# AcherStyx/SSD-Object-Detection

Hardware: AMD Instinct MI355X
Metric: images/sec SSD300 train step, batch 64 (higher is better)
Workload: dtype bf16; 1 GPU; BASELINE configs[2]: SSD300 full train step (anchor match+encode, image normalisation, conv fwd, loss, conv bwd, per-variable clip (64 variables) + Adam), per-GPU batch 64, 80 classes, synthetic COCO-shaped boxes; per_gpu_batch=64, global_batch=64, parallelism=single

## Files before the change

### ssd-object-detection_amd/csrc/conv.hip

```cpp
#include <atomic>
#include <cstdint>
#include <type_traits>
#include "common.h"
#include <hip/hip_bf16.h>
#include <stdlib.h>

#include "conv_common.h"
namespace {

template <int EPI>
__global__ void k_igemm_finalize(ConvGeom g, Epilogue ep) {
    const int n4 = (g.N + 3) >> 2;
    const long long idx = (long long)blockIdx.x * blockDim.x + threadIdx.x;
    if (idx >= (long long)g.M * n4) return;
    const int m = (int)(idx / n4), n = (int)(idx - (long long)m * n4) * 4;
    const bool full = n + 3 < g.N;
    float v[4] = {0.f, 0.f, 0.f, 0.f};
    if (full && !(g.N & 3)) {
        for (int z = 0; z < ep.ksplit; ++z) {
            const float4 t = *reinterpret_cast<const float4*>(ep.slab + ((long long)z * g.M + m) * g.N + n);
            v[0] += t.x; v[1] += t.y; v[2] += t.z; v[3] += t.w;
        }
    } else {
        for (int z = 0; z < ep.ksplit; ++z) {
// ... 362 lines not shown
    else keep_frags(fx, FW_);                                                                                       \
    __builtin_amdgcn_sched_barrier(0);                                                                              \
    __builtin_amdgcn_s_setprio(0);                                                                                  \
    if constexpr (!(ABL & 2)) __builtin_amdgcn_s_barrier();                                                              \
    __builtin_amdgcn_sched_barrier(0);

    for (int t = 0; t < nt; ++t) {
        const int cb = (t & 1) * BUF, nb = BUF - cb;
#pragma unroll
        for (int c = 0; c < 2; ++c) { fw0[c][0] = ldf(cb + OFF_W0 + wf0 + c * 2048); fw0[c][1] = ldf(cb + OFF_W0 + wf1 + c * 2048); }
        __builtin_amdgcn_sched_barrier(0);
#pragma unroll
        for (int p = 0; p < 4; ++p) { fx[p][0] = ldf(cb + OFF_X0 + xf0 + p * 2048); fx[p][1] = ldf(cb + OFF_X0 + xf1 + p * 2048); }
        __builtin_amdgcn_sched_barrier(0);
        asm volatile("s_waitcnt lgkmcnt(8)" ::: "memory");
        if constexpr (!(ABL & 1)) issue_x(nb + OFF_X1, 1);
        advance_x();
        SSD_PHASE_MMA(0, 0, fw0)
#pragma unroll
        for (int c = 0; c < 2; ++c) { fw1[c][0] = ldf(cb + OFF_W1 + wf0 + c * 2048); fw1[c][1] = ldf(cb + OFF_W1 + wf1 + c * 2048); }
        if constexpr (!(ABL & 1)) issue_w(cb + OFF_W0, 0);
        SSD_PHASE_MMA(0, 1, fw1)
#pragma unroll
        for (int p = 0; p < 4; ++p) { fx[p][0] = ldf(cb + OFF_X1 + xf0 + p * 2048); fx[p][1] = ldf(cb + OFF_X1 + xf1 + p * 2048); }
        if constexpr (!(ABL & 1)) issue_x(cb + OFF_X0, 0);
        SSD_PHASE_MMA(1, 1, fw1)
        if constexpr (!(ABL & 1)) issue_w(cb + OFF_W1, 1);
        wq += 8;
        asm volatile("s_waitcnt vmcnt(6)" ::: "memory");
        SSD_PHASE_MMA(1, 0, fw0)
    }
#undef SSD_PHASE_MMA
    if (wr == 0) __builtin_amdgcn_s_barrier();

    if (staged_ok<EPI>(g, ep) && !(g.ablate & 8)) {
        asm volatile("s_waitcnt vmcnt(0)" ::: "memory");
        auto row_to_m = [&](int row) { const int m = m0 + row; return m < g.M ? m : -1; };
        staged_epilogue<EPI, 256, 256, 4, 8, 512>(acc, smem, g, ep, n0, wr * 128, wc * 64, tid, row_to_m);
        return;
    }
    int mrow[8];
#pragma unroll
    for (int p = 0; p < 8; ++p) {
        const int m = m0 + wr * 128 + p * 16 + (lane & 15);
        mrow[p] = m < g.M ? m : -1;
    }
    conv_epilogue_rows<EPI, 4, 8>(acc, g, ep, mrow, n0 + wc * 64, lane);
}

constexpr int P32_PITCH = 96;
constexpr int P32_PATCH = 32 * 1024;
constexpr int EPI_NO_PREFETCH = 256;
constexpr int P32_OFF_MAP = 2 * P32_PATCH;

template <int BN, int EPI, bool FLAT>
__global__ __launch_bounds__(512) __attribute__((amdgpu_waves_per_eu(4, 4))) void k_conv3x3_patch32(
    const bf16_raw* __restrict__ x, const bf16_raw* __restrict__ w, ConvGeom g, Epilogue ep, int tiles_x, int tiles_y, int nblocks, int rowflat) {
    constexpr int CT = BN / 32;
    constexpr int PT = 4;
    constexpr int WBYTES = BN * 64;
    constexpr int OFF_W = 2 * P32_PATCH;
    constexpr int OFF_DUMMY = OFF_W + 2 * WBYTES;
    extern __shared__ __attribute__((aligned(16))) char smem[];

    const int tid = threadIdx.x, lane = tid & 63;
    const int wave = __builtin_amdgcn_readfirstlane(tid >> 6);
    const int wave_m = wave & 3, wave_n = wave >> 2;
    const int ntn = (g.N + BN - 1) / BN;
    const int kx = blockIdx.x >> 3;
    const int pblock = (kx / ntn) * 8 + (blockIdx.x & 7);
    if (pblock >= nblocks) return;
    const int n0 = (kx % ntn) * BN;
    constexpr bool flat = FLAT;
    const int Q = FLAT ? g.W + 1 : PATCH_W;
    const int img = (g.H + 1) * Q;
    int b = 0, y0 = 0, x0 = 0, f0 = 0;
    if constexpr (FLAT) {
        f0 = pblock * 256;
    } else {
        int t = pblock;
        const int tx = t % tiles_x; t /= tiles_x;
        x0 = tx * 16;
        if (rowflat) { y0 = t * 16; }
        else { const int ty = t % tiles_y; b = t / tiles_y; y0 = ty * 16; }
    }
    auto image_row = [&](int r) {
        if (!rowflat) { const int y = y0 + r; return (unsigned)y < (unsigned)g.H ? b * g.H + y : -1; }
        const int R = y0 + r;
        if (R < 0) return -1;
        const int bb = fdiv(R, g.d_h1), yy = R - bb * g.d_h1.d;
        return (bb < g.B && yy < g.H) ? bb * g.H + yy : -1;
    };
    auto flat_pixel = [&](int f) {
        if (f < 0) return -1;
        const int bb = f / img;
        const int r = f - bb * img;
        const int yy = r / Q, xx = r - yy * Q - 1;
        return (bb < g.B && yy < g.H && (unsigned)xx < (unsigned)g.W) ? (bb * g.H + yy) * g.W + xx : -1;
    };

    const __amdgpu_buffer_rsrc_t xres = __builtin_amdgcn_make_buffer_rsrc((void*)x, 0, (unsigned)g.B * g.H * g.W * g.C * 2u, 0x00020000);
    const __amdgpu_buffer_rsrc_t wres = __builtin_amdgcn_make_buffer_rsrc((void*)w, 0, (unsigned)g.N * (unsigned)g.ldw * 2u, 0x00020000);
    constexpr unsigned OOB = 0xfffffff0u;
    unsigned pvo[4];
#pragma unroll
    for (int j = 0; j < 4; ++j) {
// ... 102 lines not shown
            }
        }
    } else {
    dma_patch(0, 0);
    dma_w(0, 0, 0);
    for (int chunk = 0; chunk < nchunk; ++chunk) {
        const int pb = (chunk & 1) * P32_PATCH;
        const bool next_chunk = chunk + 1 < nchunk;
#pragma unroll
        for (int tap = 0; tap < 9; ++tap) {
            const int wb = ((chunk + tap) & 1) * WBYTES;
            if (tap == 1 && next_chunk) asm volatile("s_waitcnt vmcnt(4) lgkmcnt(0)" ::: "memory");
            else asm volatile("s_waitcnt vmcnt(0) lgkmcnt(0)" ::: "memory");
            __builtin_amdgcn_s_barrier();
            if (!(g.ablate & 16)) {
                if (tap < 8) dma_w(chunk, tap + 1, ((chunk + tap + 1) & 1));
                else if (next_chunk) dma_w(chunk + 1, 0, ((chunk + tap + 1) & 1));
            }
            if (tap == 0 && next_chunk && !(g.ablate & 32)) dma_patch(chunk + 1, (chunk + 1) & 1);
            bf16x8_t fx[PT], fw[CT];
            const int tapoff = pb + xbase + ((tap / 3) * Q + tap % 3) * P32_PITCH;
#pragma unroll
            for (int p = 0; p < PT; ++p) fx[p] = ldf(tapoff + p * prow);
#pragma unroll
            for (int c = 0; c < CT; ++c) fw[c] = ldf(wb + wbase + c * 1024);
            __builtin_amdgcn_s_setprio(0);
#pragma unroll
            for (int c = 0; c < CT; ++c)
#pragma unroll
                for (int p = 0; p < PT; ++p)
                    acc[c][p] = __builtin_amdgcn_mfma_f32_16x16x32_bf16(fw[c], fx[p], acc[c][p], 0, 0, 0);
            __builtin_amdgcn_s_setprio(3);
        }
    }
    }
    if (staged_ok<EPI>(g, ep) && !(g.ablate & 8)) {
        auto row_to_m = [&](int row) {
            if (flat) return flat_pixel(f0 + row);
            const int ir = image_row(row >> 4), xx = x0 + (row & 15);
            return (ir >= 0 && xx < g.Wo) ? ir * g.Wo + xx : -1;
        };
        auto pool_index = [&](int py, int px) -> long long {
            if (flat) return -1;
            int bb = b, gy = (y0 >> 1) + py;
            const int gx = (x0 >> 1) + px;
            if (rowflat) {
                const int R = y0 + 2 * py;
                bb = fdiv(R, g.d_h1);
                gy = (R - bb * g.d_h1.d) >> 1;
                if (bb >= g.B) return -1;
            }
            return (gy < ep.pool_h && gx < ep.pool_w) ? ((long long)bb * ep.pool_h + gy) * ep.pool_w + gx : -1;
        };
        if constexpr (FLAT && (BN == 128 || EPI == EPI_DGRAD)) {
            LdsSide<P32_OFF_MAP, -1, -1> side;
            side.map = side.fill = !(g.ablate & EPI_NO_PREFETCH);
            side.signs = side.bias = false;
            staged_epilogue<EPI, 256, BN, CT, PT, 512>(acc, smem, g, ep, n0, wave_m * 64, wave_n * (16 * CT), tid, row_to_m, pool_index, side);
        } else {
            staged_epilogue<EPI, 256, BN, CT, PT, 512>(acc, smem, g, ep, n0, wave_m * 64, wave_n * (16 * CT), tid, row_to_m, pool_index);
        }
        return;
    }
    int mrow[PT];
#pragma unroll
    for (int p = 0; p < PT; ++p) {
        if (flat) {
            mrow[p] = flat_pixel(f0 + (4 * wave_m + p) * 16 + (lane & 15));
        } else {
            const int ir = image_row(4 * wave_m + p), xx = x0 + (lane & 15);
            mrow[p] = (ir >= 0 && xx < g.Wo) ? ir * g.Wo + xx : -1;
        }
    }
    conv_epilogue_rows<EPI, CT, PT>(acc, g, ep, mrow, n0 + wave_n * (16 * CT), lane);
}

constexpr int P5_PIX = 34 * PATCH_W;
constexpr int P5_NDMA = (P5_PIX * 6 + 63) / 64;
constexpr int P5_PATCH = P5_NDMA * 1024;
constexpr int P5_WSLOT = 128 * 64;
constexpr int P5_OFF_W = 2 * P5_PATCH;
constexpr int P5_OFF_DUMMY = P5_OFF_W + 4 * P5_WSLOT;
constexpr int P5_LOOP_LDS = P5_OFF_DUMMY + 1024;
constexpr int P5_OFF_SIGNS = P5_LOOP_LDS;
constexpr int P5_OFF_MAP = P5_OFF_SIGNS + 512 * 16;
constexpr int P5_OFF_BIAS = P5_OFF_MAP + 512 * 4;
constexpr int P5_LDS = P5_OFF_BIAS + 128 * 4;
static_assert(P5_LDS <= 160 * 1024, "k_conv3x3_p512: LDS of one workgroup");

template <int EPI, bool FLAT>
__global__ __launch_bounds__(512) void k_conv3x3_p512(const bf16_raw* __restrict__ x, const bf16_raw* __restrict__ w, ConvGeom g,
                                                      Epilogue ep, int tiles_x, int tiles_y, int nblocks, int rowflat) {
    constexpr int BN = 128, CT = 4, PT = 8;
    extern __shared__ __attribute__((aligned(16))) char smem[];
    const int tid = threadIdx.x, lane = tid & 63;
    const int wave = __builtin_amdgcn_readfirstlane(tid >> 6);
    const int wave_m = wave & 3, wave_n = wave >> 2;
    const int ntn = (g.N + BN - 1) / BN;
    const int kx = blockIdx.x >> 3;
    const int pblock = (kx / ntn) * 8 + (blockIdx.x & 7);
    if (pblock >= nblocks) return;
    const int n0 = (kx % ntn) * BN;
    const int Q = FLAT ? g.W + 1 : PATCH_W;
    const int img = (g.H + 1) * Q;
    int b = 0, y0 = 0, x0 = 0, f0 = 0;
    if constexpr (FLAT) {
        f0 = pblock * 512;
    } else {
        int t = pblock;
        const int tx = t % tiles_x; t /= tiles_x;
        x0 = tx * 16;
        if (rowflat) { y0 = t * 32; }
        else { const int ty = t % tiles_y; b = t / tiles_y; y0 = ty * 32; }
    }
    auto image_row = [&](int r) {
        if (!rowflat) { const int y = y0 + r; return (unsigned)y < (unsigned)g.H ? b * g.H + y : -1; }
        const int R = y0 + r;
        if (R < 0) return -1;
        const int bb = fdiv(R, g.d_h1), yy = R - bb * g.d_h1.d;
        return (bb < g.B && yy < g.H) ? bb * g.H + yy : -1;
    };
    auto flat_pixel = [&](int f) {
        if (f < 0) return -1;
        const int bb = f / img;
        const int r = f - bb * img;
        const int yy = r / Q, xx = r - yy * Q - 1;
        return (bb < g.B && yy < g.H && (unsigned)xx < (unsigned)g.W) ? (bb * g.H + yy) * g.W + xx : -1;
    };
    const __amdgpu_buffer_rsrc_t xres = __builtin_amdgcn_make_buffer_rsrc((void*)x, 0, (unsigned)g.B * g.H * g.W * g.C * 2u, 0x00020000);
    const __amdgpu_buffer_rsrc_t wres = __builtin_amdgcn_make_buffer_rsrc((void*)w, 0, (unsigned)g.N * (unsigned)g.ldw * 2u, 0x00020000);
    constexpr unsigned OOB = 0xfffffff0u;
    unsigned pvo[8];
#pragma unroll
    for (int j = 0; j < 8; ++j) {
        const int q = (wave + 8 * j) * 64 + lane;
        const int pp = q / 6, sl = q - pp * 6;
        int pix;
        if constexpr (FLAT) {
            pix = pp < 512 + 2 * (Q + 1) ? flat_pixel(f0 - (Q + 1) + pp) : -1;
        } else {
            const int py = pp / PATCH_W, px = pp - py * PATCH_W;
// ... 3 lines not shown
        }
        pvo[j] = (sl < 4 && pix >= 0 && wave + 8 * j < P5_NDMA) ? ((unsigned)pix * (unsigned)g.C + (unsigned)(sl * 8)) * 2u : OOB;
    }
    unsigned wvo;
    {
        const int row = 16 * wave + (lane >> 2);
        const int piece = (lane & 3) ^ ((-(row >> 2)) & 3);
        const int n = n0 + row;
        wvo = n < g.N ? ((unsigned)n * (unsigned)g.ldw + (unsigned)(piece * 8)) * 2u : OOB;
        if (g.ablate & 16) wvo = OOB;
    }
    const int nchunk = g.C >> 5;
    const int nstep = nchunk * 9;
    auto dma_piece = [&](int chunk, int buf, int j, bool live) {
        char* dst = wave + 8 * j < P5_NDMA ? smem + buf * P5_PATCH + (wave + 8 * j) * 1024 : smem + P5_OFF_DUMMY;
        __builtin_amdgcn_raw_ptr_buffer_load_lds(xres, (lds_void*)dst, 16, live ? pvo[j] : OOB, chunk * 64, 0, 0);
    };
    auto dma_w = [&](int step) {
        const int st = step < nstep ? step : nstep - 1;
        const int ch = st / 9, tp = st - ch * 9;
        __builtin_amdgcn_raw_ptr_buffer_load_lds(wres, (lds_void*)(smem + P5_OFF_W + (step & 3) * P5_WSLOT + wave * 1024), 16, wvo,
                                                 (tp * g.C + ch * 32) * 2, 0, 0);
    };
    f32x4_t acc[CT][PT];
#pragma unroll
    for (int c = 0; c < CT; ++c)
#pragma unroll
        for (int p = 0; p < PT; ++p) acc[c][p] = f32x4_t{0.f, 0.f, 0.f, 0.f};

    const int frow = lane & 15, fk = lane >> 4;
    const int xbase = (FLAT ? 8 * wave_m * 16 + frow : 8 * wave_m * PATCH_W + frow) * P32_PITCH + fk * 16;
    constexpr int prow = (FLAT ? 16 : PATCH_W) * P32_PITCH;
    int wbase;
    {
        const int row = wave_n * 64 + frow;
        wbase = P5_OFF_W + row * 64 + ((fk ^ ((-(row >> 2)) & 3)) << 4);
    }
    auto ldf = [&](int addr) { return lds_read_b128_scoped(smem + addr, smem); };
    auto load_x = [&](bf16x8_t (&fx)[PT], int pb, int tap) {
        const int tapoff = pb + xbase + ((tap / 3) * Q + tap % 3) * P32_PITCH;
#pragma unroll
        for (int p = 0; p < PT; ++p) fx[p] = ldf(tapoff + p * prow);
    };
    auto load_w = [&](bf16x8_t (&fw)[CT], int step) {
        const int wb = (step & 3) * P5_WSLOT;
#pragma unroll
        for (int c = 0; c < CT; ++c) fw[c] = ldf(wb + wbase + c * 1024);
    };
    auto row_to_m = [&](int row) {
        if constexpr (FLAT) return flat_pixel(f0 + row);
        const int ir = image_row(row >> 4), xx = x0 + (row & 15);
        return (ir >= 0 && xx < g.Wo) ? ir * g.Wo + xx : -1;
    };
    LdsSide<P5_OFF_MAP, P5_OFF_SIGNS, P5_OFF_BIAS> side;
    side.map = side.fill = !(g.ablate & EPI_NO_PREFETCH) && staged_ok<EPI>(g, ep);
    side.signs = side.bias = false;
    if constexpr (EPI == EPI_DGRAD) {
        const long long sign_bytes = (long long)g.M * (g.N >> 3);
        side.signs = side.map && ep.mask_bits && !ep.mask_src && (g.N & 127) == 0 &&
                     (reinterpret_cast<unsigned long long>(ep.mask_bits) & 15ull) == 0 && sign_bytes < (1ll << 31) - 16;
        if (side.signs) {
            const int m = row_to_m(tid);
            lds_st4_scoped(smem + P5_OFF_MAP + tid * 4, smem, m);
            side.fill = false;
            const __amdgpu_buffer_rsrc_t sres = __builtin_amdgcn_make_buffer_rsrc((void*)ep.mask_bits, 0, (unsigned)sign_bytes, 0x00020000);
            dma16_buf(sres, smem + P5_OFF_SIGNS + wave * 1024, m >= 0 ? (unsigned)m * (unsigned)(g.N >> 3) + (unsigned)(n0 >> 3) : OOB);
        }
    } else {
        side.bias = side.map;
        if (side.bias) {
            const __amdgpu_buffer_rsrc_t bres = __builtin_amdgcn_make_buffer_rsrc((void*)ep.bias, 0, ep.bias ? (unsigned)g.N * 4u : 0u, 0x00020000);
            const int n = n0 + wave * 64 + lane;
            char* dst = wave < 2 ? smem + P5_OFF_BIAS + wave * 256 : smem + P5_OFF_DUMMY;
            __builtin_amdgcn_raw_ptr_buffer_load_lds(bres, (lds_void*)dst, 4, (wave < 2 && n < g.N) ? (unsigned)n * 4u : OOB, 0, 0, 0);
        }
    }
#pragma unroll
    for (int j = 0; j < 8; ++j) dma_piece(0, 0, j, true);
    dma_w(0); dma_w(1); dma_w(2);
    bf16x8_t fxa[PT], fxb[PT], fwa[CT], fwb[CT];
    asm volatile("s_waitcnt vmcnt(2)" ::: "memory");
    __builtin_amdgcn_s_barrier();
    load_x(fxa, 0, 0);
    load_w(fwa, 0);
    auto run_chunk = [&](int chunk, auto par_tag) {
        constexpr int PAR = decltype(par_tag)::value;
        const int pb = (chunk & 1) * P5_PATCH;
        const bool next_chunk = chunk + 1 < nchunk && !(g.ablate & 32);
#pragma unroll
        for (int tap = 0; tap < 9; ++tap) {
            constexpr int NT[9] = {1, 3, 5, 5, 5, 3, 1, 1, 1};
            if (NT[tap] == 1) asm volatile("s_waitcnt vmcnt(1) lgkmcnt(0)" ::: "memory");
            else if (NT[tap] == 3) asm volatile("s_waitcnt vmcnt(3) lgkmcnt(0)" ::: "memory");
            else asm volatile("s_waitcnt vmcnt(5) lgkmcnt(0)" ::: "memory");
            __builtin_amdgcn_s_barrier();
            const int step = chunk * 9 + tap;
            dma_w(step + 3);
            if (tap < 4) {
                dma_piece(chunk + 1, (chunk + 1) & 1, 2 * tap, next_chunk);
                dma_piece(chunk + 1, (chunk + 1) & 1, 2 * tap + 1, next_chunk);
            }
            bf16x8_t (&fxc)[PT] = ((tap + PAR) & 1) ? fxb : fxa;
            bf16x8_t (&fxn)[PT] = ((tap + PAR) & 1) ? fxa : fxb;
            bf16x8_t (&fwc)[CT] = ((tap + PAR) & 1) ? fwb : fwa;
            bf16x8_t (&fwn)[CT] = ((tap + PAR) & 1) ? fwa : fwb;
            if (tap < 8) load_x(fxn, pb, tap + 1);
            else load_x(fxn, next_chunk ? (P5_PATCH - pb) : pb, next_chunk ? 0 : 8);
            load_w(fwn, step + 1 < nstep ? step + 1 : step);
#pragma unroll
            for (int c = 0; c < CT; ++c)
// ... 1019 lines not shown
```

### ssd-object-detection_amd/csrc/conv_common.h

```cpp
#pragma once
#include <atomic>
#include <cstdint>
#include <type_traits>
#include "common.h"
#include <hip/hip_bf16.h>

namespace {

typedef __attribute__((__vector_size__(8 * sizeof(__bf16)))) __bf16 bf16x8_t;
typedef __attribute__((__vector_size__(4 * sizeof(float)))) float f32x4_t;
typedef __attribute__((__vector_size__(4 * sizeof(short)))) short s16x4_t;
typedef unsigned short bf16_raw;

constexpr int WG = 256;

struct FastDiv {
    unsigned mg;
    int sh;
    int d;
};

inline FastDiv make_fastdiv(int d) {
    FastDiv f;
    f.d = d;
// ... 166 lines not shown
#pragma unroll
        for (int j = 0; j < 4; ++j) if (n + j < N) b4[j] = ep.bias[n + j];
    }
}

template <int EPI, int CT, int PT>
__device__ __forceinline__ void conv_epilogue_rows(f32x4_t (&acc)[CT][PT], const ConvGeom& g, const Epilogue& ep,
                                                   const int (&mrow)[PT], int nbase, int lane) {
#pragma unroll
    for (int c = 0; c < CT; ++c) {
        const int n = nbase + c * 16 + (lane >> 4) * 4;
        if (n >= g.N) continue;
        const bool full = n + 3 < g.N;
        if (ep.slab) {
            float* sl = ep.slab + (long long)blockIdx.y * g.M * g.N;
#pragma unroll
            for (int p = 0; p < PT; ++p) {
                const int m = mrow[p];
                if (m < 0) continue;
                float* o = sl + (long long)m * g.N + n;
                if (full && !(g.N & 3)) {
                    *reinterpret_cast<float4*>(o) = make_float4(acc[c][p][0], acc[c][p][1], acc[c][p][2], acc[c][p][3]);
                    continue;
                }
#pragma unroll
                for (int j = 0; j < 4; ++j) if (n + j < g.N) o[j] = acc[c][p][j];
            }
            continue;
        }
        float bias4[4];
        if constexpr (EPI == EPI_DGRAD) { bias4[0] = bias4[1] = bias4[2] = bias4[3] = 0.f; }
        else load_bias4(ep, n, g.N, full, bias4);
#pragma unroll
        for (int p = 0; p < PT; ++p) {
            const int m = mrow[p];
            if (m < 0) continue;
            float v[4] = {acc[c][p][0] + bias4[0], acc[c][p][1] + bias4[1], acc[c][p][2] + bias4[2], acc[c][p][3] + bias4[3]};
            epi_store<EPI>(v, m, n, full, g, ep);
        }
    }
}

template <int EPI>
__device__ __forceinline__ bool staged_ok(const ConvGeom& g, const Epilogue& ep) {
    if (ep.slab) return false;
    if constexpr (EPI == EPI_FWD) return (g.N & 7) == 0 && (ep.ldo & 7) == 0;
    if constexpr (EPI == EPI_DGRAD) return (g.N & 7) == 0 && (ep.ldo & 7) == 0;
    return true;
}

struct NoPool { __device__ long long operator()(int, int) const { return -1; } };

struct NoSide {
    static constexpr int MAP_OFF = -1, SIGN_OFF = -1, BIAS_OFF = -1;
    bool map = false, fill = false, signs = false, bias = false;
};
template <int MAP_OFF_, int SIGN_OFF_, int BIAS_OFF_>
struct LdsSide {
    static constexpr int MAP_OFF = MAP_OFF_, SIGN_OFF = SIGN_OFF_, BIAS_OFF = BIAS_OFF_;
    bool map;
    bool fill;
    bool signs;
    bool bias;
};

__device__ __forceinline__ uint4 lds_ld16_scoped(const char* __restrict__ p, const char* __restrict__ other) {
    (void)other;
    return *reinterpret_cast<const uint4*>(p);
}
__device__ __forceinline__ void lds_st16_scoped(char* __restrict__ p, const char* __restrict__ other, uint4 v) {
    (void)other;
    *reinterpret_cast<uint4*>(p) = v;
}
__device__ __forceinline__ void lds_st8_scoped(char* __restrict__ p, const char* __restrict__ other, uint2 v) {
    (void)other;
    *reinterpret_cast<uint2*>(p) = v;
}
__device__ __forceinline__ void lds_st4_scoped(char* __restrict__ p, const char* __restrict__ other, int v) {
    (void)other;
    *reinterpret_cast<int*>(p) = v;
}
__device__ __forceinline__ bf16x8_t lds_read_b128_scoped(const char* __restrict__ p, const char* __restrict__ other) {
    (void)other;
    return *reinterpret_cast<const bf16x8_t*>(p);
}
typedef __attribute__((address_space(3))) s16x4_t lds_s16x4;
__device__ __forceinline__ s16x4_t lds_read_tr16_scoped(const char* __restrict__ p, const char* __restrict__ other) {
    (void)other;
    return __builtin_amdgcn_ds_read_tr16_b64_v4i16((lds_s16x4*)p);
}

__device__ __attribute__((aligned(16))) const unsigned g_zero16[4] = {0u, 0u, 0u, 0u};

typedef __attribute__((address_space(3))) void lds_void;
typedef __attribute__((address_space(1))) const void gbl_void;

__device__ __forceinline__ void dma16_buf(__amdgpu_buffer_rsrc_t r, char* lds, unsigned off) {
    __builtin_amdgcn_raw_ptr_buffer_load_lds(r, (lds_void*)lds, 16, off, 0, 0, 0);
}

constexpr int PATCH_W = 18;
constexpr int PATCH_PIX = PATCH_W * PATCH_W;

template <int EPI, int BM, int BN, int NT, typename RowMap, typename PoolMap, bool DG_BATCHED = true, typename Side = NoSide>
__device__ __forceinline__ void staged_store(char* smem, const ConvGeom& g, const Epilogue& ep, int n0, int tid, RowMap row_to_m_fn,
                                             PoolMap pool_index, Side side = Side{}) {
    constexpr int CPR = BN / 8;
    auto row_to_m = [&](int row) -> int {
        if constexpr (Side::MAP_OFF >= 0) {
            if (side.map) return *reinterpret_cast<const int*>(smem + Side::MAP_OFF + row * 4);
        }
        return row_to_m_fn(row);
    };
    if constexpr (EPI == EPI_HEAD) {
        const bool pairs = !((ep.per_cell | ep.level_off | ep.anchors_total | ep.n_loc | ep.n_conf) & 1);
        if (pairs) {
            constexpr int ITER2 = BM * BN / (2 * NT);
            for (int it = 0; it < ITER2; ++it) {
                const int idx = it * NT + tid;
                const int row = idx / (BN / 2), col = (idx - row * (BN / 2)) * 2;
                const int n = n0 + col;
                const int m = row_to_m(row);
                if (m < 0 || n >= ep.n_loc + ep.n_conf) continue;
                const unsigned val = *reinterpret_cast<const unsigned*>(smem + row * (BN * 2) + ((((col >> 3) ^ row) & (CPR - 1)) << 4) + (col & 7) * 2);
                const int b = fdiv(m, g.d_hw);
                const int pix = m - b * g.d_hw.d;
                const long long anchor0 = (long long)b * ep.anchors_total + ep.level_off + (long long)pix * ep.per_cell;
                if (n < ep.n_loc) *reinterpret_cast<unsigned*>(ep.loc + anchor0 * 4 + n) = val;
                else *reinterpret_cast<unsigned*>(ep.conf + anchor0 * ep.classes + (n - ep.n_loc)) = val;
            }
            return;
        }
        constexpr int ITER = BM * BN / NT;
        for (int it = 0; it < ITER; ++it) {
            const int idx = it * NT + tid;
            const int row = idx / BN, col = idx - row * BN;
            const int n = n0 + col;
            const int m = row_to_m(row);
            if (m < 0 || n >= ep.n_loc + ep.n_conf) continue;
            const bf16_raw val = *reinterpret_cast<const bf16_raw*>(smem + row * (BN * 2) + ((((col >> 3) ^ row) & (CPR - 1)) << 4) + (col & 7) * 2);
            const int b = fdiv(m, g.d_hw);
            const int pix = m - b * g.d_hw.d;
            const long long anchor0 = (long long)b * ep.anchors_total + ep.level_off + (long long)pix * ep.per_cell;
            if (n < ep.n_loc) ep.loc[anchor0 * 4 + n] = val;
            else ep.conf[anchor0 * ep.classes + (n - ep.n_loc)] = val;
        }
    } else {
        constexpr int ITER = BM * CPR / NT;
        const bool store_full = EPI != EPI_FWD || ep.out != nullptr;
        if constexpr (EPI == EPI_DGRAD && DG_BATCHED) {
            constexpr int DG_BATCH = ITER % 4 == 0 ? 4 : (ITER % 2 == 0 ? 2 : 1);
            const long long nb8 = g.N >> 3;
            bool lds_signs = false;
            if constexpr (Side::SIGN_OFF >= 0) {
                static_assert(Side::SIGN_OFF < 0 || CPR == 16, "sign table: 16 bytes per tile row");
                lds_signs = side.signs;
            }
            if (lds_signs && !ep.accumulate && !ep.up_code) {
#pragma unroll 4
                for (int it = 0; it < ITER; ++it) {
                    const int idx = it * NT + tid;
                    const int row = idx / CPR, ch = idx - row * CPR;
                    const int n = n0 + ch * 8;
                    const int m = row_to_m(row);
                    if (m < 0 || n >= g.N) continue;
                    const uint4 v = lds_ld16_scoped(smem + row * (BN * 2) + (((ch ^ row) & (CPR - 1)) << 4), smem);
                    const unsigned sb = *reinterpret_cast<const unsigned char*>(smem + Side::SIGN_OFF + idx);
                    *reinterpret_cast<uint4*>(ep.out + ((long long)m * ep.ldo + n)) = gate_bits8(v, sb);
                }
            } else
            for (int it0 = 0; it0 < ITER; it0 += DG_BATCH) {
                int mm[DG_BATCH], rr[DG_BATCH], cc[DG_BATCH];
                long long oo[DG_BATCH];
                bool ok[DG_BATCH];
#pragma unroll
                for (int j = 0; j < DG_BATCH; ++j) {
                    const int idx = (it0 + j) * NT + tid;
                    rr[j] = idx / CPR; cc[j] = idx - rr[j] * CPR;
                    const int n = n0 + cc[j] * 8;
                    mm[j] = row_to_m(rr[j]);
                    ok[j] = mm[j] >= 0 && n < g.N;
                    oo[j] = ok[j] ? (long long)mm[j] * ep.ldo + n : 0;
                }
                uint4 old[DG_BATCH], mk[DG_BATCH];
                unsigned mb[DG_BATCH], cw[DG_BATCH];
#pragma unroll
                for (int j = 0; j < DG_BATCH; ++j) { old[j] = mk[j] = make_uint4(0, 0, 0, 0); mb[j] = 0xffu; cw[j] = 0u; }
                if (ep.accumulate) {
#pragma unroll
                    for (int j = 0; j < DG_BATCH; ++j) old[j] = *reinterpret_cast<const uint4*>(ep.out + oo[j]);
                }
                if (ep.mask_src) {
#pragma unroll
                    for (int j = 0; j < DG_BATCH; ++j) mk[j] = *reinterpret_cast<const uint4*>(ep.mask_src + oo[j]);
                } else if (ep.mask_bits && !lds_signs) {
#pragma unroll
                    for (int j = 0; j < DG_BATCH; ++j) mb[j] = ep.mask_bits[ok[j] ? (long long)mm[j] * nb8 + ((n0 >> 3) + cc[j]) : 0];
                }
                if (ep.up_code) {
#pragma unroll
                    for (int j = 0; j < DG_BATCH; ++j) cw[j] = ep.up_code[ok[j] ? (long long)mm[j] * nb8 + ((n0 >> 3) + cc[j]) : 0];
                }
#pragma unroll
                for (int j = 0; j < DG_BATCH; ++j) {
                    if (!ok[j]) continue;
                    const int row = rr[j], ch = cc[j], m = mm[j];
                    const int n = n0 + ch * 8;
                    uint4 v = lds_ld16_scoped(smem + row * (BN * 2) + (((ch ^ row) & (CPR - 1)) << 4), smem);
                    if (ep.accumulate) {
                        auto add2 = [](unsigned a, unsigned b) {
                            const float lo = __uint_as_float(a << 16) + __uint_as_float(b << 16);
                            const float hi = __uint_as_float(a & 0xffff0000u) + __uint_as_float(b & 0xffff0000u);
                            return pack_bf16x2(lo, hi);
                        };
                        v.x = add2(v.x, old[j].x); v.y = add2(v.y, old[j].y); v.z = add2(v.z, old[j].z); v.w = add2(v.w, old[j].w);
                    }
                    if (ep.mask_src) {
                        auto gate = [](unsigned val, unsigned m2) {
                            if (!(__uint_as_float(m2 << 16) > 0.f)) val &= 0xffff0000u;
                            if (!(__uint_as_float(m2 & 0xffff0000u) > 0.f)) val &= 0x0000ffffu;
                            return val;
                        };
                        v.x = gate(v.x, mk[j].x); v.y = gate(v.y, mk[j].y); v.z = gate(v.z, mk[j].z); v.w = gate(v.w, mk[j].w);
                    } else if (ep.mask_bits) {
                        if (lds_signs) mb[j] = *reinterpret_cast<const unsigned char*>(smem + Side::SIGN_OFF + row * CPR + ch);
                        v = gate_bits8(v, mb[j]);
                    }
                    if (ep.up_code) {
                        const int b = fdiv(m, g.d_hw);
                        const int rem = m - b * g.d_hw.d;
                        const int oy = fdiv(rem, g.d_w), ox = rem - oy * g.d_w.d;
                        const unsigned gw[4] = {v.x, v.y, v.z, v.w};
#pragma unroll
                        for (int q = 0; q < 4; ++q) {
                            const int iy = 2 * oy + (q >> 1), ix = 2 * ox + (q & 1);
                            if (iy >= ep.up_h || ix >= ep.up_w) continue;
                            unsigned w4[4];
#pragma unroll
                            for (int k = 0; k < 4; ++k) {
                                const unsigned lo = ((cw[j] >> (8 * k)) & 15u) == (unsigned)q ? 0x0000ffffu : 0u;
                                const unsigned hi = ((cw[j] >> (8 * k + 4)) & 15u) == (unsigned)q ? 0xffff0000u : 0u;
                                w4[k] = gw[k] & (lo | hi);
                            }
                            *reinterpret_cast<uint4*>(ep.up_out + (((long long)b * ep.up_h + iy) * ep.up_w + ix) * g.N + n) =
                                make_uint4(w4[0], w4[1], w4[2], w4[3]);
                        }
                        if (!ep.out) continue;
                    }
                    *reinterpret_cast<uint4*>(ep.out + oo[j]) = v;
                }
            }
        } else
#pragma unroll 4
        for (int it = 0; it < (store_full ? ITER : 0); ++it) {
            const int idx = it * NT + tid;
            const int row = idx / CPR, ch = idx - row * CPR;
            const int n = n0 + ch * 8;
            const int m = row_to_m(row);
            if (m < 0 || n >= g.N) continue;
            uint4 v = lds_ld16_scoped(smem + row * (BN * 2) + (((ch ^ row) & (CPR - 1)) << 4), smem);
            const long long o = (long long)m * ep.ldo + n;
            if constexpr (EPI == EPI_DGRAD) {
                if (ep.accumulate) {
                    const uint4 old = *reinterpret_cast<const uint4*>(ep.out + o);
                    auto add2 = [](unsigned a, unsigned b) {
                        const float lo = __uint_as_float(a << 16) + __uint_as_float(b << 16);
                        const float hi = __uint_as_float(a & 0xffff0000u) + __uint_as_float(b & 0xffff0000u);
                        return pack_bf16x2(lo, hi);
                    };
                    v.x = add2(v.x, old.x); v.y = add2(v.y, old.y); v.z = add2(v.z, old.z); v.w = add2(v.w, old.w);
                }
                if (ep.mask_src) {
                    const uint4 mk = *reinterpret_cast<const uint4*>(ep.mask_src + o);
                    auto gate = [](unsigned val, unsigned m2) {
                        if (!(__uint_as_float(m2 << 16) > 0.f)) val &= 0xffff0000u;
                        if (!(__uint_as_float(m2 & 0xffff0000u) > 0.f)) val &= 0x0000ffffu;
                        return val;
                    };
                    v.x = gate(v.x, mk.x); v.y = gate(v.y, mk.y); v.z = gate(v.z, mk.z); v.w = gate(v.w, mk.w);
                } else if (ep.mask_bits) {
                    v = gate_bits8(v, ep.mask_bits[(long long)m * (g.N >> 3) + (n >> 3)]);
                }
            }
            if constexpr (EPI == EPI_FWD) {
                if (ep.relu_bits) ep.relu_bits[(long long)m * (g.N >> 3) + (n >> 3)] = (unsigned char)relu_bits8(v);
            }
            if constexpr (EPI == EPI_DGRAD) {
                if (ep.up_code) {
                    const int b = fdiv(m, g.d_hw);
                    const int rem = m - b * g.d_hw.d;
                    const int oy = fdiv(rem, g.d_w), ox = rem - oy * g.d_w.d;
                    const unsigned cw = ep.up_code[(long long)m * (g.N >> 3) + (n >> 3)];
                    const unsigned gw[4] = {v.x, v.y, v.z, v.w};
#pragma unroll
                    for (int q = 0; q < 4; ++q) {
                        const int iy = 2 * oy + (q >> 1), ix = 2 * ox + (q & 1);
                        if (iy >= ep.up_h || ix >= ep.up_w) continue;
                        unsigned w4[4];
#pragma unroll
// ... 38 lines not shown
                            const unsigned w0 = (&cand[0].x)[k], w1 = (&cand[1].x)[k], w2 = (&cand[2].x)[k], w3 = (&cand[3].x)[k];
                            const unsigned m = pk_max(pk_max(w0, w1), pk_max(w2, w3));
                            const unsigned ne0 = pk_min(w0 ^ m, one), ne1 = pk_min(w1 ^ m, one), ne2 = pk_min(w2 ^ m, one);
                            const unsigned t = pk_mad(ne1, ne2, ne1);
                            const unsigned first = pk_mad(ne0, t, ne0);
                            const unsigned alive = pk_min(m, one);
                            const unsigned cu = pk_mad(alive, pk_sub(first, four), four);
                            o4[k] = m;
                            cw |= ((cu & 0xfu) | ((cu >> 12) & 0xf0u)) << (8 * k);
                        }
                        *reinterpret_cast<uint4*>(ep.pool_out + po * g.N + n) = make_uint4(o4[0], o4[1], o4[2], o4[3]);
                        ep.pool_code[po * (g.N >> 3) + (n >> 3)] = cw;
                        continue;
                    }
                    float best[8];
                    unsigned pos[8];
#pragma unroll
                    for (int k = 0; k < 8; ++k) { best[k] = -INFINITY; pos[k] = 4u; }
#pragma unroll
                    for (int dy = 0; dy < 2; ++dy)
#pragma unroll
                        for (int dx = 0; dx < 2; ++dx) {
                            const int row = (2 * py + dy) * 16 + 2 * px + dx;
                            if (row_to_m(row) < 0) continue;
                            const uint4 v = lds_ld16_scoped(smem + row * (BN * 2) + (((ch ^ row) & (CPR - 1)) << 4), smem);
                            const unsigned wds[4] = {v.x, v.y, v.z, v.w};
#pragma unroll
                            for (int k = 0; k < 8; ++k) {
                                const float f = (k & 1) ? __uint_as_float(wds[k >> 1] & 0xffff0000u) : __uint_as_float(wds[k >> 1] << 16);
                                if (f > best[k]) { best[k] = f; pos[k] = (unsigned)(2 * dy + dx); }
                            }
                        }
                    unsigned o4[4], cw = 0;
#pragma unroll
                    for (int k = 0; k < 4; ++k) o4[k] = (__float_as_uint(best[2 * k]) >> 16) | (__float_as_uint(best[2 * k + 1]) & 0xffff0000u);
#pragma unroll
                    for (int k = 0; k < 8; ++k) cw |= (best[k] > 0.f ? pos[k] : 4u) << (4 * k);
                    *reinterpret_cast<uint4*>(ep.pool_out + po * g.N + n) = make_uint4(o4[0], o4[1], o4[2], o4[3]);
                    ep.pool_code[po * (g.N >> 3) + (n >> 3)] = cw;
                }
            }
        }
    }
}

template <int EPI, int BM, int BN, int CT, int PT, int NT, typename RowMap, typename PoolMap, bool DG_BATCHED = true,
          typename Side = NoSide>
__device__ __forceinline__ void staged_epilogue(f32x4_t (&acc)[CT][PT], char* smem, const ConvGeom& g, const Epilogue& ep,
                                                int n0, int wrow0, int wcol0, int tid, RowMap row_to_m, PoolMap pool_index,
                                                Side side = Side{}) {
    constexpr int CPR = BN / 8;
    const int lane = tid & 63;
    __syncthreads();
    if constexpr (Side::MAP_OFF >= 0) {
        static_assert(Side::MAP_OFF < 0 || NT >= BM, "row map: one row per thread");
        if (side.map && side.fill && tid < BM) *reinterpret_cast<int*>(smem + Side::MAP_OFF + tid * 4) = row_to_m(tid);
    }
#pragma unroll
    for (int c = 0; c < CT; ++c) {
        const int col = wcol0 + c * 16 + (lane >> 4) * 4;
        const int n = n0 + col;
        float b4[4] = {0.f, 0.f, 0.f, 0.f};
        bool lds_bias = false;
        if constexpr (Side::BIAS_OFF >= 0) lds_bias = side.bias;
        if constexpr (EPI != EPI_DGRAD) {
            if (lds_bias) {
                const float4 bv = *reinterpret_cast<const float4*>(smem + Side::BIAS_OFF + col * 4);
                b4[0] = bv.x; b4[1] = bv.y; b4[2] = bv.z; b4[3] = bv.w;
            } else if (n < g.N) load_bias4(ep, n, g.N, n + 3 < g.N, b4);
        }
#pragma unroll
        for (int p = 0; p < PT; ++p) {
            const int row = wrow0 + p * 16 + (lane & 15);
            float v[4] = {acc[c][p][0] + b4[0], acc[c][p][1] + b4[1], acc[c][p][2] + b4[2], acc[c][p][3] + b4[3]};
            if constexpr (EPI == EPI_FWD) {
                if (ep.relu) {
#pragma unroll
                    for (int j = 0; j < 4; ++j) v[j] = fmaxf(v[j], 0.f);
                }
            }
            *reinterpret_cast<uint2*>(smem + row * (BN * 2) + ((((col >> 3) ^ row) & (CPR - 1)) << 4) + (col & 4) * 2) =
                make_uint2(pack_bf16x2(v[0], v[1]), pack_bf16x2(v[2], v[3]));
        }
    }
    __syncthreads();
    staged_store<EPI, BM, BN, NT, RowMap, PoolMap, DG_BATCHED, Side>(smem, g, ep, n0, tid, row_to_m, pool_index, side);
}

template <int EPI, int BM, int BN, int CT, int PT, int NT, typename RowMap>
__device__ __forceinline__ void staged_epilogue(f32x4_t (&acc)[CT][PT], char* smem, const ConvGeom& g, const Epilogue& ep,
                                                int n0, int wrow0, int wcol0, int tid, RowMap row_to_m) {
    staged_epilogue<EPI, BM, BN, CT, PT, NT>(acc, smem, g, ep, n0, wrow0, wcol0, tid, row_to_m, NoPool{});
}

struct OnceLds { std::atomic<unsigned> done{0}; };
inline int ensure_lds(OnceLds& o, const void* fn, int bytes) {
    int dev = 0;
    if (hipGetDevice(&dev) != hipSuccess) return -1;
    const unsigned bit = 1u << (dev & 31);
    if (o.done.load(std::memory_order_acquire) & bit) return 0;
    if (hipFuncSetAttribute(fn, hipFuncAttributeMaxDynamicSharedMemorySize, bytes) != hipSuccess) return -1;
    o.done.fetch_or(bit, std::memory_order_release);
    return 0;
}

inline ConvGeom make_geom(int B, int H, int W, int C, int Ho, int Wo, int N, int KH, int KW, int mul, int div, int pad_t,
                   int pad_l) {
    ConvGeom g;
    g.B = B; g.H = H; g.W = W; g.C = C; g.Ho = Ho; g.Wo = Wo; g.N = N; g.KH = KH; g.KW = KW;
    g.mul = mul; g.div = div; g.pad_t = pad_t; g.pad_l = pad_l;
    g.M = B * Ho * Wo;
    g.nchunks = KH * KW * C / 8;
    g.ldw = KH * KW * C;
    g.cpt = C / 8;
    g.d_hw = make_fastdiv(Ho * Wo);
    g.d_w = make_fastdiv(Wo);
    g.d_h1 = make_fastdiv(H + 1);
#ifdef SSD_DEV_ABLATE
    g.ablate = ssd_knob("SSD_ABLATE", 0);
#else
    g.ablate = 0;
#endif
    g.dma32 = ((long long)B * H * W * C < (1ll << 31) - 16 && (long long)N * g.ldw < (1ll << 31) - 16) ? 1 : 0;
    g.s2 = 0;
    const int s2on = ssd_knob("SSD_DGRAD_S2", 1);
    if (div == 2 && s2on && g.cpt % 8 == 0 && KH <= 8 && KW <= 8) {
        g.s2 = 1;
        for (int p = 0; p < 2; ++p) { g.cls_h[p] = (Ho + 1 - p) / 2; g.cls_w[p] = (Wo + 1 - p) / 2; }
        for (int c = 0; c < 4; ++c) g.cls_n[c] = B * g.cls_h[c >> 1] * g.cls_w[c & 1];
    }
    return g;
}

inline bool geom_ok(int B, int H, int W, int C, int Ho, int Wo, int N, int K) {
    if (B <= 0 || H <= 0 || W <= 0 || C <= 0 || Ho <= 0 || Wo <= 0 || N <= 0 || K <= 0) return false;
    if (C % 8) return false;
// ... 16 lines not shown
```

### tools_dev/ab_conv_multi.py

```python
import sys, os
sys.path.insert(0, os.path.dirname(os.path.dirname(os.path.abspath(__file__))))
import torch
import ssd_object_detection_amd.ops as ops
from ssd_object_detection_amd import _lib
if os.environ.get('AB_LIB'):
    _lib.LIB_PATH = os.path.join(os.path.dirname(_lib.LIB_PATH), os.environ['AB_LIB'])
from tests.conv_cases import plan_name
L = _lib.lib()
for kv in os.environ.get('AB_PRESET', '').split():
    k_, v_ = kv.split('=')
    L.ssd_dev_knob(k_.encode(), int(v_))
torch.manual_seed(0)
for spec in sys.argv[1:]:
    mode, B, H, Cin, Cout, k, S, knob, vals = spec.split()
    B, H, Cin, Cout, k, S = map(int, (B, H, Cin, Cout, k, S))
    vals = [int(v) for v in vals.split(",")]
    x = torch.relu(torch.randn((B, H, H, Cin), device="cuda")).bfloat16()
    Ho, pt = ops.same_pad(H, k, S)
    cp = (Cout + 7) // 8 * 8
    if mode == "fwd":
        w = (torch.randn((Cout, k, k, Cin), device="cuda") * 0.05).bfloat16(); b = torch.zeros(Cout, device="cuda")
        y = ops.conv2d_fwd(x, w, b, S, pt, pt, Ho, Ho, True)
        run = lambda: ops.conv2d_fwd(x, w, b, S, pt, pt, Ho, Ho, True, out=y)
        plan = lambda: L.ssd_conv2d_fwd_plan(B, H, H, Cin, Cout, k, S, pt, pt, Ho, Ho, 0, 1 << 25)
    elif mode == "head":
        per_cell = Cout // 85
        w = (torch.randn((Cout, 3, 3, Cin), device="cuda") * 0.05).bfloat16(); b = torch.zeros(Cout, device="cuda")
        loc = torch.empty((B, H * H * per_cell, 4), device="cuda", dtype=torch.bfloat16)
        conf = torch.empty((B, H * H * per_cell, 81), device="cuda", dtype=torch.bfloat16)
        run = lambda: ops.conv2d_head_fwd(x, w, b, loc, conf, per_cell, 81, 0)
        plan = lambda: L.ssd_conv2d_head_fwd_plan(B, H, H, Cin, per_cell, 81, 1 << 25)
    elif mode == "wgrad":
        dy = torch.zeros((B, Ho, Ho, cp), device="cuda").bfloat16(); dy[..., :Cout] = torch.randn((B, Ho, Ho, Cout), device="cuda").bfloat16()
        dw, db = ops.conv2d_bwd_weight(x, dy, Cout, k, S, pt, pt)
        run = lambda: ops.conv2d_bwd_weight(x, dy, Cout, k, S, pt, pt, dw=dw, dbias=db)
        plan = lambda: L.ssd_conv2d_bwd_weight_plan(B, H, H, Cin, Cout, cp, k, S, pt, pt, Ho, Ho)
    elif mode == "w0fused":
        dy = torch.randn((B, H, H, 64), device="cuda").bfloat16()
        w_t = (torch.randn((64, 3, 3, 64), device="cuda") * 0.05).bfloat16()
        img = torch.zeros((B, H, H, 8), device="cuda").bfloat16(); img[..., :3] = torch.randn((B, H, H, 3), device="cuda").bfloat16()
        bits = torch.randint(0, 256, (B, H, H, 8), device="cuda", dtype=torch.uint8)
        dw, db = ops.conv2d_bwd_data_wgrad_first(dy, w_t, bits, img)
        run = lambda: ops.conv2d_bwd_data_wgrad_first(dy, w_t, bits, img, dw=dw, dbias=db)
        plan = lambda: -1
    elif mode == "dgradbits":
        dy = torch.zeros((B, Ho, Ho, cp), device="cuda").bfloat16(); dy[..., :Cout] = torch.randn((B, Ho, Ho, Cout), device="cuda").bfloat16()
        w_t = (torch.randn((Cin, k, k, cp), device="cuda") * 0.05).bfloat16()
        dx = torch.empty((B, H, H, Cin), device="cuda", dtype=torch.bfloat16)
        bits = torch.randint(0, 256, (B, H, H, Cin // 8), device="cuda", dtype=torch.uint8)
        run = lambda: ops.conv2d_bwd_data_bits(dy, w_t, bits, (B, H, H, Cin), S, pt, pt, accumulate=False, out=dx)
        plan = lambda: L.ssd_conv2d_bwd_data_plan(B, H, H, Cin, cp, k, S, pt, pt, Ho, Ho, 0, 1 << 25)
    else:
        dy = torch.zeros((B, Ho, Ho, cp), device="cuda").bfloat16(); dy[..., :Cout] = torch.randn((B, Ho, Ho, Cout), device="cuda").bfloat16()
        w_t = (torch.randn((Cin, k, k, cp), device="cuda") * 0.05).bfloat16()
        dx = torch.empty((B, H, H, Cin), device="cuda", dtype=torch.bfloat16)
        run = lambda: ops.conv2d_bwd_data(dy, w_t, x, (B, H, H, Cin), S, pt, pt, accumulate=False, out=dx)
        plan = lambda: L.ssd_conv2d_bwd_data_plan(B, H, H, Cin, cp, k, S, pt, pt, Ho, Ho, 0, 1 << 25)

    def timed(v, reps=10):
        L.ssd_dev_knob(knob.encode(), v)
        run(); torch.cuda.synchronize()
        e0, e1 = torch.cuda.Event(enable_timing=True), torch.cuda.Event(enable_timing=True)
        e0.record()
        for _ in range(reps):
            run()
        e1.record(); torch.cuda.synchronize()
        return e0.elapsed_time(e1) / reps * 1e3
    t = {v: [] for v in vals}
    for rnd in range(5):
        for v in vals:
            t[v].append(timed(v))
    fl = 2.0 * B * Ho * Ho * Cout * k * k * Cin
    out = []
    for v in vals:
        L.ssd_dev_knob(knob.encode(), v)
        a = sorted(t[v])
        out.append("%s=%d [%s] %.1f us %.0f TF/s" % (knob, v, (plan_name(L, plan()) if plan() >= 0 else "fused"), a[len(a) // 2], fl / a[len(a) // 2] / 1e6))
    L.ssd_dev_knob(knob.encode(), vals[0])
    print("%-5s B%d %dx%d %d->%d k%d s%d: " % (mode, B, H, H, Cin, Cout, k, S) + " | ".join(out), flush=True)
```

Measured before the change: 7435 images/sec.

## Precompute un-pool row table and late-load sign bits in LDS for dgrad epilogues

Adds an LDS table of per-row un-pool base offsets and boundary flags, built once per tile so the dgrad+unpool epilogue no longer recomputes fast divisions for every stored chunk. In the patch32 dgrad kernel, the mask sign bits are now DMA'd into LDS during the epilogue, overlapping with accumulator staging. The p512 kernel also gets the un-pool table, placed in the weight ring region. This adds LDS aliasing and wait-count complexity, plus a small table-build cost per tile.

```diff
diff --git a/ssd-object-detection_amd/csrc/conv.hip b/ssd-object-detection_amd/csrc/conv.hip
--- a/ssd-object-detection_amd/csrc/conv.hip
+++ b/ssd-object-detection_amd/csrc/conv.hip
@@ -438,6 +438,9 @@
 constexpr int P32_PATCH = 32 * 1024;
 constexpr int EPI_NO_PREFETCH = 256;
 constexpr int P32_OFF_MAP = 2 * P32_PATCH;
+constexpr int P32_OFF_UP = P32_OFF_MAP + 1024;
+constexpr int P32_OFF_SIGNS = P32_OFF_MAP + 2048;
+static_assert(P32_OFF_SIGNS + 256 * 16 <= 2 * P32_PATCH + 2 * 128 * 64, "patch32: side tables");
 
 template <int BN, int EPI, bool FLAT>
 __global__ __launch_bounds__(512) __attribute__((amdgpu_waves_per_eu(4, 4))) void k_conv3x3_patch32(
@@ -646,7 +649,18 @@
             }
             return (gy < ep.pool_h && gx < ep.pool_w) ? ((long long)bb * ep.pool_h + gy) * ep.pool_w + gx : -1;
         };
-        if constexpr (FLAT && (BN == 128 || EPI == EPI_DGRAD)) {
+        if constexpr (EPI == EPI_DGRAD) {
+            LdsSide<P32_OFF_MAP, P32_OFF_SIGNS, -1, P32_OFF_UP, true> side;
+            const bool pre = !(g.ablate & EPI_NO_PREFETCH);
+            const long long rows8 = (long long)g.M * (g.N >> 3);
+            side.map = side.fill = pre && FLAT;
+            side.bias = false;
+            side.signs = pre && ep.mask_bits && !ep.mask_src && g.N % BN == 0 &&
+                         (reinterpret_cast<unsigned long long>(ep.mask_bits) & 15ull) == 0 && rows8 < (1ll << 31) - 16;
+            side.up = pre && unpool_table_ok(g, ep);
+            const int etid = FLAT ? wave * 64 + (int)__builtin_amdgcn_mbcnt_hi(~0u, __builtin_amdgcn_mbcnt_lo(~0u, 0u)) : tid;
+            staged_epilogue<EPI, 256, BN, CT, PT, 512>(acc, smem, g, ep, n0, wave_m * 64, wave_n * (16 * CT), etid, row_to_m, pool_index, side);
+        } else if constexpr (FLAT && BN == 128) {
             LdsSide<P32_OFF_MAP, -1, -1> side;
             side.map = side.fill = !(g.ablate & EPI_NO_PREFETCH);
             side.signs = side.bias = false;
@@ -681,6 +695,8 @@
 constexpr int P5_OFF_BIAS = P5_OFF_MAP + 512 * 4;
 constexpr int P5_LDS = P5_OFF_BIAS + 128 * 4;
 static_assert(P5_LDS <= 160 * 1024, "k_conv3x3_p512: LDS of one workgroup");
+constexpr int P5_OFF_UP = 512 * 128 * 2;
+static_assert(P5_OFF_UP >= P5_OFF_W && P5_OFF_UP + 512 * 4 <= P5_LOOP_LDS, "k_conv3x3_p512: un-pool row table in the weight ring");
 
 template <int EPI, bool FLAT>
 __global__ __launch_bounds__(512) void k_conv3x3_p512(const bf16_raw* __restrict__ x, const bf16_raw* __restrict__ w, ConvGeom g,
@@ -790,10 +806,11 @@
         const int ir = image_row(row >> 4), xx = x0 + (row & 15);
         return (ir >= 0 && xx < g.Wo) ? ir * g.Wo + xx : -1;
     };
-    LdsSide<P5_OFF_MAP, P5_OFF_SIGNS, P5_OFF_BIAS> side;
+    LdsSide<P5_OFF_MAP, P5_OFF_SIGNS, P5_OFF_BIAS, P5_OFF_UP> side;
     side.map = side.fill = !(g.ablate & EPI_NO_PREFETCH) && staged_ok<EPI>(g, ep);
     side.signs = side.bias = false;
     if constexpr (EPI == EPI_DGRAD) {
+        side.up = side.map && unpool_table_ok(g, ep);
         const long long sign_bytes = (long long)g.M * (g.N >> 3);
         side.signs = side.map && ep.mask_bits && !ep.mask_src && (g.N & 127) == 0 &&
                      (reinterpret_cast<unsigned long long>(ep.mask_bits) & 15ull) == 0 && sign_bytes < (1ll << 31) - 16;
diff --git a/ssd-object-detection_amd/csrc/conv_common.h b/ssd-object-detection_amd/csrc/conv_common.h
--- a/ssd-object-detection_amd/csrc/conv_common.h
+++ b/ssd-object-detection_amd/csrc/conv_common.h
@@ -242,17 +242,23 @@
 struct NoPool { __device__ long long operator()(int, int) const { return -1; } };
 
 struct NoSide {
-    static constexpr int MAP_OFF = -1, SIGN_OFF = -1, BIAS_OFF = -1;
-    bool map = false, fill = false, signs = false, bias = false;
+    static constexpr int MAP_OFF = -1, SIGN_OFF = -1, BIAS_OFF = -1, UP_OFF = -1;
+    static constexpr bool LATE = false;
+    bool map = false, fill = false, signs = false, bias = false, up = false;
 };
-template <int MAP_OFF_, int SIGN_OFF_, int BIAS_OFF_>
+template <int MAP_OFF_, int SIGN_OFF_, int BIAS_OFF_, int UP_OFF_ = -1, bool LATE_ = false>
 struct LdsSide {
-    static constexpr int MAP_OFF = MAP_OFF_, SIGN_OFF = SIGN_OFF_, BIAS_OFF = BIAS_OFF_;
+    static constexpr int MAP_OFF = MAP_OFF_, SIGN_OFF = SIGN_OFF_, BIAS_OFF = BIAS_OFF_, UP_OFF = UP_OFF_;
+    static constexpr bool LATE = LATE_;
     bool map;
     bool fill;
     bool signs;
     bool bias;
+    bool up = false;
 };
+__device__ __forceinline__ bool unpool_table_ok(const ConvGeom& g, const Epilogue& ep) {
+    return ep.up_code && (long long)g.B * ep.up_h * ep.up_w <= (1ll << 30);
+}
 
 __device__ __forceinline__ uint4 lds_ld16_scoped(const char* __restrict__ p, const char* __restrict__ other) {
     (void)other;
@@ -342,10 +348,37 @@
             constexpr int DG_BATCH = ITER % 4 == 0 ? 4 : (ITER % 2 == 0 ? 2 : 1);
             const long long nb8 = g.N >> 3;
             bool lds_signs = false;
-            if constexpr (Side::SIGN_OFF >= 0) {
-                static_assert(Side::SIGN_OFF < 0 || CPR == 16, "sign table: 16 bytes per tile row");
-                lds_signs = side.signs;
-            }
+            if constexpr (Side::SIGN_OFF >= 0) lds_signs = side.signs;
+            bool lds_up = false;
+            if constexpr (Side::UP_OFF >= 0) lds_up = side.up;
+            auto unpool = [&](const uint4& v, unsigned cw, int m, int row, int n) {
+                long long base;
+                bool y1, x1;
+                if (lds_up) {
+                    const unsigned e = *reinterpret_cast<const unsigned*>(smem + (Side::UP_OFF >= 0 ? Side::UP_OFF : 0) + row * 4);
+                    base = e >> 2; y1 = e & 2u; x1 = e & 1u;
+                } else {
+                    const int b = fdiv(m, g.d_hw);
+                    const int rem = m - b * g.d_hw.d;
+                    const int oy = fdiv(rem, g.d_w), ox = rem - oy * g.d_w.d;
+                    base = ((long long)b * ep.up_h + 2 * oy) * ep.up_w + 2 * ox;
+                    y1 = 2 * oy + 1 < ep.up_h; x1 = 2 * ox + 1 < ep.up_w;
+                }
+                const unsigned gw[4] = {v.x, v.y, v.z, v.w};
+#pragma unroll
+                for (int q = 0; q < 4; ++q) {
+                    if (((q >> 1) && !y1) || ((q & 1) && !x1)) continue;
+                    unsigned w4[4];
+#pragma unroll
+                    for (int k = 0; k < 4; ++k) {
+                        const unsigned lo = ((cw >> (8 * k)) & 15u) == (unsigned)q ? 0x0000ffffu : 0u;
+                        const unsigned hi = ((cw >> (8 * k + 4)) & 15u) == (unsigned)q ? 0xffff0000u : 0u;
+                        w4[k] = gw[k] & (lo | hi);
+                    }
+                    *reinterpret_cast<uint4*>(ep.up_out + (base + (q >> 1) * ep.up_w + (q & 1)) * g.N + n) =
+                        make_uint4(w4[0], w4[1], w4[2], w4[3]);
+                }
+            };
             if (lds_signs && !ep.accumulate && !ep.up_code) {
 #pragma unroll 4
                 for (int it = 0; it < ITER; ++it) {
@@ -355,7 +388,7 @@
                     const int m = row_to_m(row);
                     if (m < 0 || n >= g.N) continue;
                     const uint4 v = lds_ld16_scoped(smem + row * (BN * 2) + (((ch ^ row) & (CPR - 1)) << 4), smem);
-                    const unsigned sb = *reinterpret_cast<const unsigned char*>(smem + Side::SIGN_OFF + idx);
+                    const unsigned sb = *reinterpret_cast<const unsigned char*>(smem + (Side::SIGN_OFF >= 0 ? Side::SIGN_OFF : 0) + idx);
                     *reinterpret_cast<uint4*>(ep.out + ((long long)m * ep.ldo + n)) = gate_bits8(v, sb);
                 }
             } else
@@ -413,28 +446,11 @@
                         };
                         v.x = gate(v.x, mk[j].x); v.y = gate(v.y, mk[j].y); v.z = gate(v.z, mk[j].z); v.w = gate(v.w, mk[j].w);
                     } else if (ep.mask_bits) {
-                        if (lds_signs) mb[j] = *reinterpret_cast<const unsigned char*>(smem + Side::SIGN_OFF + row * CPR + ch);
+                        if (lds_signs) mb[j] = *reinterpret_cast<const unsigned char*>(smem + (Side::SIGN_OFF >= 0 ? Side::SIGN_OFF : 0) + row * CPR + ch);
                         v = gate_bits8(v, mb[j]);
                     }
                     if (ep.up_code) {
-                        const int b = fdiv(m, g.d_hw);
-                        const int rem = m - b * g.d_hw.d;
-                        const int oy = fdiv(rem, g.d_w), ox = rem - oy * g.d_w.d;
-                        const unsigned gw[4] = {v.x, v.y, v.z, v.w};
-#pragma unroll
-                        for (int q = 0; q < 4; ++q) {
-                            const int iy = 2 * oy + (q >> 1), ix = 2 * ox + (q & 1);
-                            if (iy >= ep.up_h || ix >= ep.up_w) continue;
-                            unsigned w4[4];
-#pragma unroll
-                            for (int k = 0; k < 4; ++k) {
-                                const unsigned lo = ((cw[j] >> (8 * k)) & 15u) == (unsigned)q ? 0x0000ffffu : 0u;
-                                const unsigned hi = ((cw[j] >> (8 * k + 4)) & 15u) == (unsigned)q ? 0xffff0000u : 0u;
-                                w4[k] = gw[k] & (lo | hi);
-                            }
-                            *reinterpret_cast<uint4*>(ep.up_out + (((long long)b * ep.up_h + iy) * ep.up_w + ix) * g.N + n) =
-                                make_uint4(w4[0], w4[1], w4[2], w4[3]);
-                        }
+                        unpool(v, cw[j], m, row, n);
                         if (!ep.out) continue;
                     }
                     *reinterpret_cast<uint4*>(ep.out + oo[j]) = v;
@@ -579,9 +595,51 @@
     constexpr int CPR = BN / 8;
     const int lane = tid & 63;
     __syncthreads();
+    if constexpr (Side::LATE && EPI == EPI_DGRAD) {
+        __builtin_amdgcn_s_waitcnt(0x0F70);
+    }
     if constexpr (Side::MAP_OFF >= 0) {
         static_assert(Side::MAP_OFF < 0 || NT >= BM, "row map: one row per thread");
-        if (side.map && side.fill && tid < BM) *reinterpret_cast<int*>(smem + Side::MAP_OFF + tid * 4) = row_to_m(tid);
+        bool up = false;
+        if constexpr (Side::UP_OFF >= 0 && EPI == EPI_DGRAD) up = side.up;
+        if (((side.map && side.fill) || up) && tid < BM) {
+            const int m = (side.map && !side.fill) ? *reinterpret_cast<const int*>(smem + Side::MAP_OFF + tid * 4) : row_to_m(tid);
+            if (side.map && side.fill) *reinterpret_cast<int*>(smem + Side::MAP_OFF + tid * 4) = m;
+            if constexpr (Side::UP_OFF >= 0 && EPI == EPI_DGRAD) {
+                if (up) {
+                    unsigned e = 0;
+                    if (m >= 0) {
+                        const int b = fdiv(m, g.d_hw);
+                        const int rem = m - b * g.d_hw.d;
+                        const int oy = fdiv(rem, g.d_w), ox = rem - oy * g.d_w.d;
+                        e = ((unsigned)((b * ep.up_h + 2 * oy) * ep.up_w + 2 * ox) << 2) | (2 * oy + 1 < ep.up_h ? 2u : 0u) |
+                            (2 * ox + 1 < ep.up_w ? 1u : 0u);
+                    }
+                    *reinterpret_cast<unsigned*>(smem + Side::UP_OFF + tid * 4) = e;
+                }
+            }
+        }
+    }
+    if constexpr (Side::LATE && EPI == EPI_DGRAD) {
+        static_assert(!Side::LATE || (BM == 256 && NT == 512 && (BN == 128 || BN == 64)), "late side tables: k_conv3x3_patch32's tile");
+        constexpr unsigned OOB = 0xfffffff0u;
+        const int wave = __builtin_amdgcn_readfirstlane(tid >> 6);
+        const unsigned nb8 = (unsigned)(g.N >> 3);
+        if constexpr (Side::SIGN_OFF >= 0) {
+            if (side.signs) {
+                const __amdgpu_buffer_rsrc_t sres = __builtin_amdgcn_make_buffer_rsrc((void*)ep.mask_bits, 0, (unsigned)g.M * nb8, 0x00020000);
+                if constexpr (BN == 128) {
+                    if (wave < 4) {
+                        const int m = row_to_m(tid);
+                        dma16_buf(sres, smem + Side::SIGN_OFF + wave * 1024, m >= 0 ? (unsigned)m * nb8 + (unsigned)(n0 >> 3) : OOB);
+                    }
+                } else {
+                    const int m = row_to_m(tid >> 1);
+                    __builtin_amdgcn_raw_ptr_buffer_load_lds(sres, (lds_void*)(smem + Side::SIGN_OFF + wave * 256), 4,
+                                                             m >= 0 ? (unsigned)m * nb8 + (unsigned)(n0 >> 3) + (unsigned)(tid & 1) * 4u : OOB, 0, 0, 0);
+                }
+            }
+        }
     }
 #pragma unroll
     for (int c = 0; c < CT; ++c) {
@@ -606,9 +664,14 @@
                     for (int j = 0; j < 4; ++j) v[j] = fmaxf(v[j], 0.f);
                 }
             }
-            *reinterpret_cast<uint2*>(smem + row * (BN * 2) + ((((col >> 3) ^ row) & (CPR - 1)) << 4) + (col & 4) * 2) =
-                make_uint2(pack_bf16x2(v[0], v[1]), pack_bf16x2(v[2], v[3]));
-        }
+            char* dst = smem + row * (BN * 2) + ((((col >> 3) ^ row) & (CPR - 1)) << 4) + (col & 4) * 2;
+            const uint2 pk = make_uint2(pack_bf16x2(v[0], v[1]), pack_bf16x2(v[2], v[3]));
+            if constexpr (Side::LATE && EPI == EPI_DGRAD) lds_st8_scoped(dst, smem, pk);
+            else *reinterpret_cast<uint2*>(dst) = pk;
+        }
+    }
+    if constexpr (Side::LATE && EPI == EPI_DGRAD) {
+        if (side.signs) asm volatile("s_waitcnt vmcnt(0)" ::: "memory");
     }
     __syncthreads();
     staged_store<EPI, BM, BN, NT, RowMap, PoolMap, DG_BATCHED, Side>(smem, g, ep, n0, tid, row_to_m, pool_index, side);
diff --git a/tools_dev/ab_conv_multi.py b/tools_dev/ab_conv_multi.py
--- a/tools_dev/ab_conv_multi.py
+++ b/tools_dev/ab_conv_multi.py
@@ -50,6 +50,14 @@
         bits = torch.randint(0, 256, (B, H, H, Cin // 8), device="cuda", dtype=torch.uint8)
         run = lambda: ops.conv2d_bwd_data_bits(dy, w_t, bits, (B, H, H, Cin), S, pt, pt, accumulate=False, out=dx)
         plan = lambda: L.ssd_conv2d_bwd_data_plan(B, H, H, Cin, cp, k, S, pt, pt, Ho, Ho, 0, 1 << 25)
+    elif mode == "dgradunpool":
+        Hf = 2 * H - (H == 38)
+        full = torch.randn((B, Hf, Hf, Cin), device="cuda").bfloat16()
+        _, code = ops.maxpool2x2_fwd_argmax(full, same=True)
+        dy = torch.zeros((B, H, H, cp), device="cuda").bfloat16(); dy[..., :Cout] = torch.randn((B, H, H, Cout), device="cuda").bfloat16()
+        w_t = (torch.randn((Cin, 3, 3, cp), device="cuda") * 0.05).bfloat16()
+        run = lambda: ops.conv2d_bwd_data_unpool(dy, w_t, None, code, (B, Hf, Hf, Cin), out=full)
+        plan = lambda: L.ssd_conv2d_bwd_data_unpool_plan(B, H, H, Cin, cp, Hf, Hf, 0, 1 << 25)
     else:
         dy = torch.zeros((B, Ho, Ho, cp), device="cuda").bfloat16(); dy[..., :Cout] = torch.randn((B, Ho, Ho, Cout), device="cuda").bfloat16()
         w_t = (torch.randn((Cin, k, k, cp), device="cuda") * 0.05).bfloat16()
diff --git a/tools_dev/step_launch_medians.py b/tools_dev/step_launch_medians.py
--- /dev/null
+++ b/tools_dev/step_launch_medians.py
@@ -0,0 +1,27 @@
+import csv, glob, re, statistics, sys
+args = sys.argv[1:]
+skip = 5
+if args[0] == '--skip':
+    skip = int(args[1]); args = args[2:]
+def short(n):
+    n = n.replace('(anonymous namespace)::', '').replace('void ', '')
+    return re.sub(r'\(.*', '', n)[:40]
+def medians(d):
+    f = glob.glob(d + '/**/*_kernel_trace.csv', recursive=True)[0]
+    rows = sorted(csv.DictReader(open(f)), key=lambda r: int(r['Start_Timestamp']))
+    starts = [i for i, r in enumerate(rows) if 'k_image_prep' in r['Kernel_Name']] + [len(rows)]
+    per = {}
+    for a, b in list(zip(starts[:-1], starts[1:]))[skip:]:
+        seen = {}
+        for r in rows[a:b]:
+            k = (short(r['Kernel_Name']), r['Grid_Size_X'])
+            seen[k] = seen.get(k, 0) + 1
+            per.setdefault(k + (seen[k],), []).append((int(r['End_Timestamp']) - int(r['Start_Timestamp'])) / 1e3)
+    return {k: (statistics.median(v), len(v)) for k, v in per.items()}
+tabs = [medians(d) for d in args]
+keys = sorted(tabs[0], key=lambda k: -tabs[0][k][0])
+print('%-42s %9s %3s  ' % ('kernel', 'grid', '#') + ' '.join('%9s' % d.rstrip('/').split('/')[-1][-9:] for d in args))
+for k in keys:
+    v = [t.get(k, (float('nan'), 0))[0] for t in tabs]
+    print('%-42s %9s %3d  ' % k + ' '.join('%9.1f' % x for x in v))
+print('%-42s %9s %3s  ' % ('sum of medians', '', '') + ' '.join('%9.1f' % sum(t[k][0] for k in t) for t in tabs))
```

Result: no change. 7455 images/sec (median of 6 runs) (+0.3%).
